# leimao/Voice-Converter-CycleGAN

Measured on NVIDIA H100. Metric: CycleGAN-VC train steps/sec @ batch 256x[24,128] MCEP, higher is better.
Workload: dtype f16f8 (forward / data gradient: fp16 MMA + two e4m3 cross-term MMAs = 2 MMA units per product; weight gradient: fp16 MMA alone, 1 unit; f32 accumulate)

## Files before the change

### voice-converter-cyclegan_b200/csrc/tc_gemm.cu

```cuda
#include "tc_gemm.cuh"
#include "geom.h"
#include "kernels.cuh"
#include "wgmma.cuh"

#include <cuda.h>
#include <stdint.h>
#include <stdio.h>

namespace {

typedef CUresult (*EncodeTiledFn)(CUtensorMap*, CUtensorMapDataType, cuuint32_t, void*, const cuuint64_t*, const cuuint64_t*,
                                  const cuuint32_t*, const cuuint32_t*, CUtensorMapInterleave, CUtensorMapSwizzle,
                                  CUtensorMapL2promotion, CUtensorMapFloatOOBfill);
EncodeTiledFn get_encoder() {
  static EncodeTiledFn fn = nullptr;
  if (!fn) {
    void* p = nullptr; cudaDriverEntryPointQueryResult q;
    if (cudaGetDriverEntryPoint("cuTensorMapEncodeTiled", &p, cudaEnableDefault, &q) == cudaSuccess && q == cudaDriverEntryPointSuccess)
      fn = (EncodeTiledFn)p;
  }
  return fn;
}
bool make_tmap3(CUtensorMap* m, const void* base, uint64_t d0, uint64_t d1, uint64_t d2, uint32_t b1) {
  EncodeTiledFn enc = get_encoder();
  if (!enc) return false;
  cuuint64_t dims[3] = {d0, d1, d2};
  cuuint64_t strides[2] = {d0 * 2, d0 * d1 * 2};
  cuuint32_t box[3] = {64, b1, 1};
  cuuint32_t es[3] = {1, 1, 1};
  return enc(m, CU_TENSOR_MAP_DATA_TYPE_BFLOAT16, 3, const_cast<void*>(base), dims, strides, box, es, CU_TENSOR_MAP_INTERLEAVE_NONE,
             CU_TENSOR_MAP_SWIZZLE_128B, CU_TENSOR_MAP_L2_PROMOTION_L2_256B, CU_TENSOR_MAP_FLOAT_OOB_FILL_NONE) == CUDA_SUCCESS;
}

bool make_tmap3_t(CUtensorMap* m, const void* base, CUtensorMapDataType dt, int esize, uint64_t d0, uint64_t d1, uint64_t d2, uint32_t b0, uint32_t b1) {
  EncodeTiledFn enc = get_encoder();
  if (!enc) return false;
  cuuint64_t dims[3] = {d0, d1, d2};
  cuuint64_t strides[2] = {d0 * (uint64_t)esize, d0 * d1 * (uint64_t)esize};
  cuuint32_t box[3] = {b0, b1, 1};
  cuuint32_t es[3] = {1, 1, 1};
  return enc(m, dt, 3, const_cast<void*>(base), dims, strides, box, es, CU_TENSOR_MAP_INTERLEAVE_NONE,
             b0 * esize == 64 ? CU_TENSOR_MAP_SWIZZLE_64B : CU_TENSOR_MAP_SWIZZLE_128B, CU_TENSOR_MAP_L2_PROMOTION_L2_256B,
             CU_TENSOR_MAP_FLOAT_OOB_FILL_NONE) == CUDA_SUCCESS;
}

__device__ __forceinline__ uint32_t smem_u32(const void* p) { return (uint32_t)__cvta_generic_to_shared(p); }

__device__ __forceinline__ void mbar_init(uint64_t* bar, uint32_t count) {
  asm volatile("mbarrier.init.shared::cta.b64 [%0], %1;" ::"r"(smem_u32(bar)), "r"(count));
}
__device__ __forceinline__ void fence_barrier_init() { asm volatile("fence.mbarrier_init.release.cluster;" ::: "memory"); }
__device__ __forceinline__ void mbar_wait(uint64_t* bar, uint32_t parity) {
  asm volatile(
      "{\n\t"
      ".reg .pred p;\n\t"
      "WAIT_LOOP:\n\t"
      "mbarrier.try_wait.parity.shared::cta.b64 p, [%0], %1;\n\t"
      "@p bra.uni WAIT_DONE;\n\t"
      "bra.uni WAIT_LOOP;\n\t"
      "WAIT_DONE:\n\t"
      "}" ::"r"(smem_u32(bar)), "r"(parity) : "memory");
}
__device__ __forceinline__ void cp_async16(uint32_t dst_smem, const void* src, uint32_t src_bytes) {
  asm volatile("cp.async.cg.shared.global [%0], [%1], 16, %2;" ::"r"(dst_smem), "l"(src), "r"(src_bytes) : "memory");
}
__device__ __forceinline__ void cp_async_arrive_noinc(uint64_t* bar) {
  asm volatile("cp.async.mbarrier.arrive.noinc.shared::cta.b64 [%0];" ::"r"(smem_u32(bar)) : "memory");
}
__device__ __forceinline__ void mbar_expect_tx(uint64_t* bar, uint32_t bytes) {
  asm volatile("mbarrier.arrive.expect_tx.shared::cta.b64 _, [%0], %1;" ::"r"(smem_u32(bar)), "r"(bytes) : "memory");
}
__device__ __forceinline__ void tma_load3(uint32_t dst_smem, const CUtensorMap* map, int c0, int c1, int c2, uint64_t* bar) {
  asm volatile("cp.async.bulk.tensor.3d.shared::cluster.global.tile.mbarrier::complete_tx::bytes [%0], [%1, {%2, %3, %4}], [%5];"
               ::"r"(dst_smem), "l"(map), "r"(c0), "r"(c1), "r"(c2), "r"(smem_u32(bar)) : "memory");
}
__device__ __forceinline__ void tma_prefetch_desc(const CUtensorMap* map) {
  asm volatile("prefetch.tensormap [%0];" ::"l"(map) : "memory");
}
__device__ __forceinline__ void fence_proxy_async() { asm volatile("fence.proxy.async.shared::cta;" ::: "memory"); }
__device__ __forceinline__ uint64_t make_desc(uint32_t smem_addr, uint32_t lbo_bytes, uint32_t sbo_bytes, uint64_t layout = 1) {
  return (uint64_t)((smem_addr >> 4) & 0x3FFF) | ((uint64_t)((lbo_bytes >> 4) & 0x3FFF) << 16) |
         ((uint64_t)((sbo_bytes >> 4) & 0x3FFF) << 32) | (layout << 62);
}
__device__ __forceinline__ uint64_t make_desc64(uint32_t smem_addr) { return make_desc(smem_addr, 16, 512, 2); }
template <int N>
__device__ __forceinline__ void fence_acc(float (&d)[N]) {
#pragma unroll
  for (int i = 0; i < N; ++i) asm volatile("" : "+f"(d[i])::"memory");
}
__device__ __forceinline__ void mbar_arrive(uint64_t* bar) {
  asm volatile("mbarrier.arrive.shared::cta.b64 _, [%0];" ::"r"(smem_u32(bar)) : "memory");
}
__device__ __forceinline__ void consumer_bar() { asm volatile("bar.sync 3, 256;" ::: "memory"); }
__device__ __forceinline__ void st_shared16(uint32_t addr, uint4 v) {
  asm volatile("st.shared.v4.b32 [%0], {%1, %2, %3, %4};" ::"r"(addr), "r"(v.x), "r"(v.y), "r"(v.z), "r"(v.w) : "memory");
}
__device__ __forceinline__ uint4 e4m3x8_to_f16x8(uint2 v) {
  uint32_t w[4];
#pragma unroll
  for (int i = 0; i < 4; ++i) {
    const uint32_t src = (i < 2 ? v.x : v.y) >> (16 * (i & 1));
    const __half2_raw h = __nv_cvt_fp8x2_to_halfraw2((__nv_fp8x2_storage_t)(src & 0xFFFFu), __NV_E4M3);
    w[i] = (uint32_t)h.x | ((uint32_t)h.y << 16);
  }
  return make_uint4(w[0], w[1], w[2], w[3]);
}

struct FastDiv { uint32_t mul, shr, d; };
__host__ inline FastDiv make_fastdiv(uint32_t d) {
  FastDiv f; f.d = d;
  uint32_t l = 0; while ((1ull << l) < d) ++l;
  f.mul = (uint32_t)(((1ull << 32) * ((1ull << l) - d)) / d + 1);
  f.shr = l;
  return f;
}
__device__ __forceinline__ uint32_t fdiv(uint32_t n, const FastDiv& f) { return (uint32_t)(((uint64_t)__umulhi(n, f.mul) + n) >> f.shr); }

__device__ __forceinline__ uint32_t sw128(int r, int c) { return (uint32_t)((r >> 3) * 1024 + (r & 7) * 128 + ((c ^ (r & 7)) << 4)); }

struct TcNTParams {
  GatherGeom g;
  const __nv_bfloat16 *a_hi, *a_lo; int a_ld; int C;
  const __nv_bfloat16 *b_hi, *b_lo; int Nw;
  int N;
  int n_tiles;
  int debug;
  float* dst; int d_ld; const float* bias; int accumulate;
  int perm; int Cc;
  int R;
  const float *gamma_a, *beta_a, *gamma_g, *beta_g;
  float* stats;
  const float* resid;
  float* y; __nv_bfloat16 *y_hi, *y_lo;
  int C_out;
  const float* bp; int bp_ld;
  __nv_bfloat16 *dp_hi, *dp_lo; int dp_ld;
  float *dbeta_a, *dgamma_a, *dbeta_g, *dgamma_g;
  CUtensorMap tm_b_hi, tm_b_lo;
  const uint8_t *a8_hi, *a8_lo;
  CUtensorMap tm_b8_hi, tm_b8_lo;
  uint8_t* y8;
  PackGeom pk;
  FastDiv div_bw, div_w;
};

struct RowPos { int b, y, x; };
__device__ __forceinline__ RowPos nt_row(const TcNTParams& p, long long m) {
  RowPos r;
  r.y = (int)fdiv((uint32_t)m, p.div_bw);
  const uint32_t rem = (uint32_t)m - (uint32_t)r.y * p.div_bw.d;
  r.b = (int)fdiv(rem, p.div_w);
  r.x = (int)(rem - (uint32_t)r.b * p.div_w.d);
  return r;
}
__device__ __forceinline__ uint32_t nt_tile_taps(const TcNTParams& p, long long m0, long long M) {
  const long long m1 = m0 + 127 < M ? m0 + 127 : M - 1;
  return gather_tap_mask(p.g, nt_row(p, m0).y, nt_row(p, m1).y);
}

struct TcTNParams {
  GatherGeom g;
  const __nv_bfloat16 *x_hi, *x_lo; int x_ld; int C;
  const __nv_bfloat16 *g_hi, *g_lo; int g_ld; int N;
  float* dw_a; float* dw_g; int n_split;
  int ksplit;
  FastDiv div_hw, div_w;
  CUtensorMap tm_g_hi, tm_g_lo;
  const uint8_t *x8_hi, *x8_lo;
  const uint8_t *g8_hi, *g8_lo;
  int w16;
  int fold_n;
  float* part; long long part_k, numel_a;
};

__device__ __forceinline__ float* tn_dst(float* base, int slab, int C, int c, int ncols, int col, int fold_n) {
  if (fold_n) { const int t = col / fold_n; return base + ((long long)t * C + c) * fold_n + (col - t * fold_n); }
  return base + ((long long)slab * C + c) * ncols + col;
}

constexpr int kProducerThreads = 128;


template <int BN, int NPL>
struct NTCfg {
  static constexpr int A_PLANE = 128 * 128;
  static constexpr int B_PLANE = BN * 128;
  static constexpr int PLANES = NPL == 2 ? 2 : 1;
  static constexpr int STAGE = PLANES * (A_PLANE + B_PLANE);
  static constexpr int STAGES = (192 * 1024) / STAGE;
  static constexpr int SMEM = STAGES * STAGE + 1024;
  static_assert(STAGES * STAGE >= 128 * BN * 4, "the finished fp32 tile is staged over the pipeline stages");
};

template <int BN>
__device__ __forceinline__ int acc_off(int r, int n) { return r * BN + (n & ~31) + ((((n >> 2) & 7) ^ (r & 7)) << 2) + (n & 3); }
template <int BN>
__device__ __forceinline__ void acc_ld32(const float* acc, int r, int col, uint32_t (&v)[32]) {
#pragma unroll
  for (int c = 0; c < 8; ++c) {
    const float4 x = *reinterpret_cast<const float4*>(acc + r * BN + col + ((c ^ (r & 7)) << 2));
    v[4 * c] = __float_as_uint(x.x); v[4 * c + 1] = __float_as_uint(x.y); v[4 * c + 2] = __float_as_uint(x.z); v[4 * c + 3] = __float_as_uint(x.w);
  }
}

__device__ __forceinline__ float warp_colsum32(float (&t)[32], int lane) {
#pragma unroll
  for (int o = 16, n = 32; o >= 1; o >>= 1, n >>= 1) {
    const bool up = (lane & o) != 0;
#pragma unroll
    for (int i = 0; i < n / 2; ++i) {
      float send = up ? t[i] : t[i + n / 2];
      float keep = up ? t[i + n / 2] : t[i];
      t[i] = keep + __shfl_xor_sync(0xffffffffu, send, o);
    }
  }
  return t[0];
}
__device__ __forceinline__ void epi_bar(int id) { asm volatile("bar.sync %0, 128;" ::"r"(id) : "memory"); }

__device__ __forceinline__ float sample_sum(float v, float (*xch)[32], int q, int lane, int spw, int barid) {
  if (spw == 1) return v;
  epi_bar(barid);
  xch[q][lane] = v;
  epi_bar(barid);
  const int q0 = (q / spw) * spw;
  float r = 0.f;
  for (int w = 0; w < spw; ++w) r += xch[q0 + w][lane];
  return r;
}
__device__ __forceinline__ void bc4(const float* p, float (&v)[4]) { const float4 x = *reinterpret_cast<const float4*>(p); v[0] = x.x; v[1] = x.y; v[2] = x.z; v[3] = x.w; }
__device__ __forceinline__ float fast_sigmoid(float x) { return __fdividef(1.f, 1.f + __expf(-x)); }
__device__ __forceinline__ void chunk_norm_coeffs(const float (&v)[32], const float* __restrict__ gamma, const float* __restrict__ beta,
                                                  int ch, int R, float (*xch)[32], float* bc, int q, int lane, int spw, int barid, float& mean, float& rstd) {
  float t[32];
#pragma unroll
  for (int k = 0; k < 32; ++k) t[k] = v[k];
  float s = warp_colsum32(t, lane);
  s = sample_sum(s, xch, q, lane, spw, barid);
  mean = s / (float)R;
  __syncwarp();
  bc[lane] = mean;
  __syncwarp();
#pragma unroll
  for (int k = 0; k < 32; k += 4) {
    float4 m4 = *reinterpret_cast<const float4*>(bc + k);
    float d0 = v[k] - m4.x, d1 = v[k + 1] - m4.y, d2 = v[k + 2] - m4.z, d3 = v[k + 3] - m4.w;
    t[k] = d0 * d0; t[k + 1] = d1 * d1; t[k + 2] = d2 * d2; t[k + 3] = d3 * d3;
  }
  float ss = warp_colsum32(t, lane);
  ss = sample_sum(ss, xch, q, lane, spw, barid);
  rstd = 1.f / sqrtf(ss / (float)R + 1e-6f);
  const float sc = rstd * gamma[ch + lane];
  const float of = beta[ch + lane] - mean * sc;
  __syncwarp();
  bc[lane] = sc; bc[32 + lane] = of;
  __syncwarp();
}

__device__ __forceinline__ void pair_norm_coeffs(const float (&v0)[32], const float (&v1)[32], const float* __restrict__ gamma, const float* __restrict__ beta,
                                                 int ch, int R, float (*xch)[32], float* bc, int q, int lane, int spw, int barid, float& mean, float& rstd) {
  float t[32];
#pragma unroll
  for (int k = 0; k < 32; ++k) t[k] = v0[k] + v1[k];
  float s = warp_colsum32(t, lane);
  s = sample_sum(s, xch, q, lane, spw, barid);
  const float inv = 1.f / (float)(2 * R);
  mean = s * inv;
  __syncwarp();
  bc[lane] = mean;
  __syncwarp();
#pragma unroll
  for (int k = 0; k < 32; k += 4) {
    float4 m4 = *reinterpret_cast<const float4*>(bc + k);
    const float m[4] = {m4.x, m4.y, m4.z, m4.w};
#pragma unroll
    for (int j = 0; j < 4; ++j) { const float d0 = v0[k + j] - m[j], d1 = v1[k + j] - m[j]; t[k + j] = fmaf(d0, d0, d1 * d1); }
  }
  float ss = warp_colsum32(t, lane);
  ss = sample_sum(ss, xch, q, lane, spw, barid);
  rstd = 1.f / sqrtf(ss * inv + 1e-6f);
  const float sc = rstd * gamma[ch + lane];
  const float of = beta[ch + lane] - mean * sc;
  __syncwarp();
  bc[lane] = sc; bc[32 + lane] = of;
  __syncwarp();
}

__device__ __forceinline__ uint32_t hp_off(int r, int c) { return (uint32_t)(r * 16 + ((c ^ ((r >> 1) & 3)) << 2)); }
template <class F>
__device__ __forceinline__ void rows_out(float* stg, const float (&o)[32], int lane, F f) {
  const int hc = lane & 3, hr = lane >> 2;
#pragma unroll
  for (int h = 0; h < 2; ++h) {
    __syncwarp();
#pragma unroll
    for (int c = 0; c < 4; ++c)
      *reinterpret_cast<float4*>(stg + hp_off(lane, c)) = make_float4(o[16 * h + 4 * c], o[16 * h + 4 * c + 1], o[16 * h + 4 * c + 2], o[16 * h + 4 * c + 3]);
    __syncwarp();
#pragma unroll
    for (int i = 0; i < 4; ++i) {
      const int rr = hr + 8 * i;
      f(rr, 16 * h + 4 * hc, *reinterpret_cast<const float4*>(stg + hp_off(rr, hc)));
    }
  }
}
__device__ __forceinline__ void rows_in(float* stg, float (&v)[32], int lane, const float4 (&pre)[8]) {
  const int hc = lane & 3, hr = lane >> 2;
#pragma unroll
  for (int h = 0; h < 2; ++h) {
    __syncwarp();
#pragma unroll
    for (int i = 0; i < 4; ++i) *reinterpret_cast<float4*>(stg + hp_off(hr + 8 * i, hc)) = pre[4 * h + i];
    __syncwarp();
#pragma unroll
    for (int c = 0; c < 4; ++c) {
      const float4 x = *reinterpret_cast<const float4*>(stg + hp_off(lane, c));
      v[16 * h + 4 * c] = x.x; v[16 * h + 4 * c + 1] = x.y; v[16 * h + 4 * c + 2] = x.z; v[16 * h + 4 * c + 3] = x.w;
    }
// ... 454 lines not shown
  const bool n_fast = g.Hy > 1;

  if (threadIdx.x == 0) {
    for (int s = 0; s < S; ++s) { mbar_init(&full_bar[s], kProducerThreads + 1); mbar_init(&empty_bar[s], 8); }
    mbar_init(&acc_free_bar, 8);
    fence_barrier_init();
    tma_prefetch_desc(&p.tm_b_hi);
    if (NPL == 2) tma_prefetch_desc(&p.tm_b_lo);
    if (NPL == 3) { tma_prefetch_desc(&p.tm_b8_hi); tma_prefetch_desc(&p.tm_b8_lo); }
  }
  __syncthreads();

  if (warp < 4) {
    const int t = threadIdx.x;
    const int chunk = t & 7, rsub = t >> 3;
    int stage = 0; uint32_t phase = 0;
    int it = 0;
    for (int tile = blockIdx.x; tile < num_tiles; tile += gridDim.x, ++it) {
      const long long m0 = (long long)(n_fast ? tile / n_tiles : tile % m_tiles) * 128;
      const int n0 = (n_fast ? tile % n_tiles : tile / m_tiles) * BN;
      if (EPI != 0 && it > 0) mbar_wait(&acc_free_bar, (uint32_t)(it - 1) & 1u);
      const uint32_t taps = nt_tile_taps(p, m0, M);
      int rb[8], ry[8], rx[8];
#pragma unroll
      for (int i = 0; i < 8; ++i) {
        long long m = m0 + rsub + 16 * i;
        if (m < M) {
          if constexpr (PK) {
            const int dout = p.pk.div * g.sx;
            const int u = pack_find(p.pk.off, p.pk.n, m * dout);
            const long long o0 = __ldg(p.pk.off + u), o1 = __ldg(p.pk.off + u + 1);
            rb[i] = (int)(o0 / p.pk.div); ry[i] = (int)((o1 - o0) / p.pk.div); rx[i] = (int)(m - o0 / dout) * g.sx;
          } else {
            const RowPos o = nt_row(p, m);
            rb[i] = o.b; ry[i] = o.y * g.sy; rx[i] = o.x * g.sx;
          }
        } else { rb[i] = -1; ry[i] = 0; rx[i] = 0; }
      }
      for (int pass = 0; pass < (NPL == 3 ? 2 : 1); ++pass)
      for (int tap = 0; tap < g.ntaps; ++tap) {
        if (!((taps >> tap) & 1u)) continue;
        long long aoff[8];
#pragma unroll
        for (int i = 0; i < 8; ++i) {
          const int cofs = NPL == 3 && pass == 0 ? (chunk & 3) * 16 : chunk * 8;
          if constexpr (PK) {
            const int xx = rx[i] + g.ox[tap];
            aoff[i] = rb[i] >= 0 && xx >= 0 && xx < ry[i] ? (long long)(rb[i] + xx) * p.a_ld + cofs : -1;
          } else {
            int yy = ry[i] + g.oy[tap], xx = rx[i] + g.ox[tap];
            bool ok = rb[i] >= 0 && yy >= 0 && yy < g.Hs && xx >= 0 && xx < g.Ws;
            aoff[i] = ok ? ((long long)(rb[i] * g.Hs + yy) * g.Ws + xx) * p.a_ld + cofs : -1;
          }
        }
        for (int cc = 0; cc < cchunks; ++cc) {
          const int c0 = cc << 6;
          mbar_wait(&empty_bar[stage], phase ^ 1);
          const uint32_t sA = smem_base + stage * Cfg::STAGE;
          const uint32_t sB = sA + Cfg::PLANES * Cfg::A_PLANE;
          if (t == 0) {
            mbar_expect_tx(&full_bar[stage], Cfg::PLANES * Cfg::B_PLANE);
            if (NPL == 3) {
              if (pass == 0) {
                tma_load3(sB, &p.tm_b8_hi, c0, n0, g.widx[tap], &full_bar[stage]);
                tma_load3(sB + Cfg::B_PLANE / 2, &p.tm_b8_lo, c0, n0, g.widx[tap], &full_bar[stage]);
              } else {
                tma_load3(sB, &p.tm_b_hi, c0, n0, g.widx[tap], &full_bar[stage]);
              }
            } else {
              tma_load3(sB, &p.tm_b_hi, c0, n0, g.widx[tap], &full_bar[stage]);
              if (NPL == 2) tma_load3(sB + Cfg::B_PLANE, &p.tm_b_lo, c0, n0, g.widx[tap], &full_bar[stage]);
            }
          }
          if (!(p.debug & 4)) {
#pragma unroll
            for (int i = 0; i < 8; ++i) {
              const int r = rsub + 16 * i;
              const uint32_t so = sw128(r, chunk);
              const bool ok = aoff[i] >= 0;
              const long long off = ok ? aoff[i] + c0 : 0;
              if (NPL == 3) {
                if (pass == 0)
                  cp_async16(sA + so, (chunk < 4 ? p.a8_hi : p.a8_lo) + off, ok ? 16u : 0u);
                else
                  cp_async16(sA + so, p.a_hi + off, ok ? 16u : 0u);
              } else {
                cp_async16(sA + so, p.a_hi + off, ok ? 16u : 0u);
                if (NPL == 2) cp_async16(sA + Cfg::A_PLANE + so, p.a_lo + off, ok ? 16u : 0u);
              }
            }
          }
          cp_async_arrive_noinc(&full_bar[stage]);
          if (++stage == S) { stage = 0; phase ^= 1; }
        }
      }
    }
  } else {
    const int cw = warp - 4;
    const int wg = cw >> 2;
    const int tw = threadIdx.x - 128 * (wg + 1);
    float* acc_s = reinterpret_cast<float*>(smem_raw + (smem_base - smem_u32(smem_raw)));
    int stage = 0; uint32_t phase = 0;
    for (int tile = blockIdx.x; tile < num_tiles; tile += gridDim.x) {
      const long long m0 = (long long)(n_fast ? tile / n_tiles : tile % m_tiles) * 128;
      const int n0 = (n_fast ? tile % n_tiles : tile / m_tiles) * BN;
      float d[BN / 2];
#pragma unroll
      for (int i = 0; i < BN / 2; ++i) d[i] = 0.f;
      int prev = -1;
      const int kb_pass = __popc(nt_tile_taps(p, m0, M)) * cchunks;
      if constexpr (NPL == 3) {
        consume_stages<BN, MMA_E4M3_CROSS, 0, Cfg>(d, kb_pass, stage, phase, prev, full_bar, empty_bar, smem_base, wg, lane);
        rescale_acc(d, 1.f / (float)(1 << CGVC_Q_ACC_SHIFT));
        consume_stages<BN, MMA_F16, 0, Cfg>(d, kb_pass, stage, phase, prev, full_bar, empty_bar, smem_base, wg, lane);
      } else {
        consume_stages<BN, NPL == 2 ? MMA_BF16X3 : MMA_BF16, 0, Cfg>(d, kb_pass, stage, phase, prev, full_bar, empty_bar, smem_base, wg, lane);
      }
      wgmma_wait<0>();
      fence_acc(d);
      if (prev >= 0 && lane == 0) mbar_arrive(&empty_bar[prev]);
      const int r0 = wg * 64 + (tw >> 5) * 16 + ((tw & 31) >> 2), c0 = 2 * (tw & 3);
      if constexpr (EPI == 0) {
        if (!(p.debug & 3)) nt_store_fragments<BN>(p, d, M, m0, n0, r0, c0);
      } else {
        consumer_bar();
        if (!(p.debug & 2)) {
#pragma unroll
          for (int j = 0; j < BN / 8; ++j) {
            *reinterpret_cast<float2*>(acc_s + acc_off<BN>(r0, 8 * j + c0)) = make_float2(d[4 * j], d[4 * j + 1]);
            *reinterpret_cast<float2*>(acc_s + acc_off<BN>(r0 + 8, 8 * j + c0)) = make_float2(d[4 * j + 2], d[4 * j + 3]);
          }
        }
        consumer_bar();
        nt_tile_epilogue<BN, NPL, EPI>(p, M, m0, n0, cw & 3, lane, epi_stage[cw], epi_rowp[cw], epi_bc[cw], epi_xch[wg], acc_s, wg, 2);
        fence_proxy_async();
        __syncwarp();
        if (lane == 0) mbar_arrive(&acc_free_bar);
      }
    }
  }
}

#define CGVC_Q_WGRAD_SHIFT 12
template <int NPL, int W16>
struct TNCfg {
  static constexpr int A_PLANE = 64 * 256;
  static constexpr int B_PLANE = 64 * 512;
  static constexpr int PLANES = (NPL == 1 || W16) ? 1 : 2;
  static constexpr int STAGE = PLANES * (A_PLANE + B_PLANE);
  static constexpr int STAGES = (192 * 1024) / STAGE;
  static constexpr int SMEM = STAGES * STAGE + 1024;
};

template <int NPL, int W16, int DET>
__global__ void __launch_bounds__(kNTThreads, 1)
tc_gg_tn_kernel(const __grid_constant__ TcTNParams p) {
  static_assert(W16 == 0 || NPL == 3, "the fp16-only weight gradient is a form of CGVC_PREC_F16F8");
  using Cfg = TNCfg<NPL, W16>;
  constexpr int S = Cfg::STAGES;
  constexpr int BN = 256;
  extern __shared__ uint8_t smem_raw[];
  __shared__ __align__(8) uint64_t full_bar[S], empty_bar[S];

  const uint32_t smem_base = (smem_u32(smem_raw) + 1023u) & ~1023u;
  const int warp = threadIdx.x >> 5, lane = threadIdx.x & 31;
  const GatherGeom& g = p.g;
  const long long M = (long long)g.B * g.Hy * g.Wx;
  const int HW = g.Hy * g.Wx;
  const int n_tiles = (p.g_ld + BN - 1) / BN, c_tiles = (p.x_ld + 127) / 128;
  const int num_items = n_tiles * c_tiles * g.ntaps * p.ksplit;
  constexpr int pass0 = (NPL == 3 && !W16) ? 0 : 1;
  long long chunk_rows = (M + p.ksplit - 1) / p.ksplit;
  chunk_rows = (chunk_rows + 63) / 64 * 64;

  struct Item { int n0, c0, tap, ks; long long mbeg, mend; int num_kb; };
  auto decode = [&](int item) -> Item {
    Item w;
    int n_t = item % n_tiles; int t1 = item / n_tiles;
    int c_t = t1 % c_tiles; int t2 = t1 / c_tiles;
    w.tap = t2 % g.ntaps; const int ks = t2 / g.ntaps; w.ks = ks;
    w.n0 = n_t * BN; w.c0 = c_t * 128;
    w.mbeg = (long long)ks * chunk_rows;
    w.mend = (w.mbeg + chunk_rows < M) ? w.mbeg + chunk_rows : M;
    w.num_kb = w.mend > w.mbeg ? (int)((w.mend - w.mbeg + 63) / 64) : 0;
    return w;
  };

  if (threadIdx.x == 0) {
    for (int s = 0; s < S; ++s) { mbar_init(&full_bar[s], kProducerThreads + 1); mbar_init(&empty_bar[s], 8); }
    fence_barrier_init();
    tma_prefetch_desc(&p.tm_g_hi);
    if (NPL == 2) tma_prefetch_desc(&p.tm_g_lo);
  }
  __syncthreads();

  if (warp < 4) {
    const int t = threadIdx.x;
    const int chunk = t & 7, rsub = t >> 3;
    int stage = 0; uint32_t phase = 0;
    for (int item = blockIdx.x; item < num_items; item += gridDim.x) {
      const Item w = decode(item);
      for (int pass = pass0; pass < 2; ++pass)
      for (int kb = 0; kb < w.num_kb; ++kb) {
        mbar_wait(&empty_bar[stage], phase ^ 1);
        const uint32_t sA = smem_base + stage * Cfg::STAGE;
        const uint32_t sB = sA + Cfg::PLANES * Cfg::A_PLANE;
        long long xoff[4];
#pragma unroll
        for (int i = 0; i < 4; ++i) {
          const long long m = w.mbeg + (long long)kb * 64 + rsub + 16 * i;
          xoff[i] = -1;
          if (m < w.mend) {
            const uint32_t mu = (uint32_t)m;
            int b = (int)fdiv(mu, p.div_hw); int rem = (int)(mu - (uint32_t)b * (uint32_t)HW);
            int y = (int)fdiv((uint32_t)rem, p.div_w); int x = rem - y * g.Wx;
            int yy = y * g.sy + g.oy[w.tap], xx = x * g.sx + g.ox[w.tap];
            if (yy >= 0 && yy < g.Hs && xx >= 0 && xx < g.Ws)
              xoff[i] = ((long long)(b * g.Hs + yy) * g.Ws + xx) * p.x_ld + w.c0 + chunk * 8;
          }
        }
        if (NPL == 3 && pass == 0) {
#pragma unroll
          for (int i = 0; i < 4; ++i) {
            const int kr = rsub + 16 * i;
            const uint32_t so = sw128(kr, chunk);
#pragma unroll
            for (int a = 0; a < 2; ++a) {
              const bool ok = xoff[i] >= 0 && (w.c0 + a * 64) < p.x_ld;
              uint2 vh = make_uint2(0u, 0u), vl = make_uint2(0u, 0u);
              if (ok) { vh = __ldg(reinterpret_cast<const uint2*>(p.x8_hi + xoff[i] + a * 64)); vl = __ldg(reinterpret_cast<const uint2*>(p.x8_lo + xoff[i] + a * 64)); }
              st_shared16(sA + a * 8192 + so, e4m3x8_to_f16x8(vh));
              st_shared16(sA + Cfg::A_PLANE + a * 8192 + so, e4m3x8_to_f16x8(vl));
            }
            const long long m = w.mbeg + (long long)kb * 64 + kr;
#pragma unroll
            for (int a = 0; a < 4; ++a) {
              const int col = w.n0 + a * 64 + chunk * 8;
              const bool ok = m < w.mend && col < p.g_ld;
              uint2 vh = make_uint2(0u, 0u), vl = make_uint2(0u, 0u);
              if (ok) { vh = __ldg(reinterpret_cast<const uint2*>(p.g8_hi + m * p.g_ld + col)); vl = __ldg(reinterpret_cast<const uint2*>(p.g8_lo + m * p.g_ld + col)); }
              st_shared16(sB + a * 8192 + so, e4m3x8_to_f16x8(vh));
              st_shared16(sB + Cfg::B_PLANE + a * 8192 + so, e4m3x8_to_f16x8(vl));
            }
          }
          fence_proxy_async();
          if (t == 0) mbar_expect_tx(&full_bar[stage], 0);
          mbar_arrive(&full_bar[stage]);
        } else {
          if (t == 0) {
            const int row0 = (int)(w.mbeg + (long long)kb * 64);
            int natoms = 0;
#pragma unroll
            for (int a = 0; a < 4; ++a) natoms += (w.n0 + a * 64) < p.g_ld ? 1 : 0;
            mbar_expect_tx(&full_bar[stage], (NPL == 2 ? 2 : 1) * natoms * 8192);
#pragma unroll
            for (int a = 0; a < 4; ++a) {
              if ((w.n0 + a * 64) < p.g_ld) {
                tma_load3(sB + a * 8192, &p.tm_g_hi, w.n0 + a * 64, row0, 0, &full_bar[stage]);
                if (NPL == 2) tma_load3(sB + Cfg::B_PLANE + a * 8192, &p.tm_g_lo, w.n0 + a * 64, row0, 0, &full_bar[stage]);
              }
            }
          }
#pragma unroll
          for (int i = 0; i < 4; ++i) {
            const uint32_t so = sw128(rsub + 16 * i, chunk);
#pragma unroll
            for (int a = 0; a < 2; ++a) {
              const bool ok = xoff[i] >= 0 && (w.c0 + a * 64) < p.x_ld;
              const long long off = ok ? xoff[i] + a * 64 : 0;
              cp_async16(sA + a * 8192 + so, p.x_hi + off, ok ? 16u : 0u);
              if (NPL == 2) cp_async16(sA + Cfg::A_PLANE + a * 8192 + so, p.x_lo + off, ok ? 16u : 0u);
            }
          }
          cp_async_arrive_noinc(&full_bar[stage]);
        }
        if (++stage == S) { stage = 0; phase ^= 1; }
      }
    }
  } else {
    const int cw = warp - 4;
    const int wg = cw >> 2;
    const int tw = threadIdx.x - 128 * (wg + 1);
    int stage = 0; uint32_t phase = 0;
    for (int item = blockIdx.x; item < num_items; item += gridDim.x) {
      const Item w = decode(item);
      if (w.num_kb == 0) continue;
      float d[BN / 2];
#pragma unroll
      for (int i = 0; i < BN / 2; ++i) d[i] = 0.f;
      int prev = -1;
      if constexpr (NPL == 3 && !W16) {
        consume_stages<BN, MMA_F16_CROSS, 1, Cfg>(d, w.num_kb, stage, phase, prev, full_bar, empty_bar, smem_base, wg, lane);
        rescale_acc(d, 1.f / (float)(1 << CGVC_Q_WGRAD_SHIFT));
        consume_stages<BN, MMA_F16, 1, Cfg>(d, w.num_kb, stage, phase, prev, full_bar, empty_bar, smem_base, wg, lane);
      } else if constexpr (NPL == 3) {
        consume_stages<BN, MMA_F16, 1, Cfg>(d, w.num_kb, stage, phase, prev, full_bar, empty_bar, smem_base, wg, lane);
      } else {
        consume_stages<BN, NPL == 2 ? MMA_BF16X3 : MMA_BF16, 1, Cfg>(d, w.num_kb, stage, phase, prev, full_bar, empty_bar, smem_base, wg, lane);
      }
      wgmma_wait<0>();
      fence_acc(d);
      if (lane == 0) mbar_arrive(&empty_bar[prev]);
      const int c = w.c0 + wg * 64 + (tw >> 5) * 16 + ((tw & 31) >> 2);
#pragma unroll
      for (int j = 0; j < BN / 8; ++j) {
        const int n = w.n0 + 8 * j + 2 * (tw & 3);
        if (n >= p.N) continue;
        float* base; int nn; int ncols;
        if (n < p.n_split) { base = DET ? p.part + w.ks * p.part_k : p.dw_a; nn = n; ncols = p.n_split; }
        else { base = DET ? p.part + w.ks * p.part_k + p.numel_a : p.dw_g; nn = n - p.n_split; ncols = p.N - p.n_split; }
#pragma unroll
        for (int h = 0; h < 2; ++h) {
          if (c + 8 * h >= p.C) continue;
          float* dst = tn_dst(base, g.widx[w.tap], p.C, c + 8 * h, ncols, nn, p.fold_n);
          if constexpr (DET) asm volatile("st.global.v2.f32 [%0], {%1, %2};" ::"l"(dst), "f"(d[4 * j + 2 * h]), "f"(d[4 * j + 2 * h + 1]) : "memory");
          else asm volatile("red.global.add.v2.f32 [%0], {%1, %2};" ::"l"(dst), "f"(d[4 * j + 2 * h]), "f"(d[4 * j + 2 * h + 1]) : "memory");
        }
      }
    }
  }
}

__host__ __device__ __forceinline__ int perm_row(int perm, int co, int cout, int noff) {
  if (perm == 1) return (co >> 7) * 256 + (noff ? 128 : 0) + (co & 127);
  if (perm == 2) { const int Ch = cout >> 1; const int s = co >= Ch ? 1 : 0; const int c = co - s * Ch; return (c >> 6) * 256 + (noff ? 128 : 0) + s * 64 + (c & 63); }
  return noff + co;
}
__host__ __device__ __forceinline__ long long w_src(int tap, int ci, int co, int cin, int cout, int fold_n) {
  if (fold_n) { const int t = co / fold_n; return ((long long)t * cin + ci) * fold_n + (co - t * fold_n); }
  return ((long long)tap * cin + ci) * cout + co;
}
__global__ void __launch_bounds__(256)
prep_weights_kernel(const float* __restrict__ w, int taps, int cin, int cout, int nt_n, int cin_k, int cin_n, int nt_k, int noff, int perm, int fold_n,
                    __nv_bfloat16* __restrict__ wf_hi, __nv_bfloat16* __restrict__ wf_lo,
                    __nv_bfloat16* __restrict__ wd_hi, __nv_bfloat16* __restrict__ wd_lo) {
  __shared__ float tile[32][33];
  const int tap = blockIdx.z;
  const int ci0 = blockIdx.y * 32, co0 = blockIdx.x * 32;
  const int tx = threadIdx.x & 31, ty = threadIdx.x >> 5;
  for (int r = ty; r < 32; r += 8) {
    int ci = ci0 + r, co = co0 + tx;
    float v = 0.f;
    if (ci < cin && co < cout) {
      v = w[w_src(tap, ci, co, cin, cout, fold_n)];
      __nv_bfloat16 h = __float2bfloat16_rn(v);
      __nv_bfloat16 l = __float2bfloat16_rn(v - __bfloat162float(h));
      long long o = ((long long)tap * cin_n + ci) * nt_k + noff + co;
      wd_hi[o] = h; wd_lo[o] = l;
    }
    tile[r][tx] = v;
  }
  __syncthreads();
  for (int r = ty; r < 32; r += 8) {
    int co = co0 + r, ci = ci0 + tx;
    if (ci < cin && co < cout) {
      float v = tile[tx][r];
      __nv_bfloat16 h = __float2bfloat16_rn(v);
      __nv_bfloat16 l = __float2bfloat16_rn(v - __bfloat162float(h));
      const int nrow = perm_row(perm, co, cout, noff);
      long long o = ((long long)tap * nt_n + nrow) * cin_k + ci;
      wf_hi[o] = h; wf_lo[o] = l;
    }
  }
}

__global__ void copy_bias_kernel(const float* __restrict__ b, float* __restrict__ dst, int n, int noff, int perm) {
  int i = blockIdx.x * 256 + threadIdx.x;
  if (i < n) dst[perm_row(perm, i, n, noff)] = b[i];
}

__global__ void __launch_bounds__(256)
prep_weights_q_kernel(const float* __restrict__ w, int taps, int cin, int cout, int nt_n, int cin_q, int noff, int perm, int fold_n,
                      __half* __restrict__ q16, uint8_t* __restrict__ q8hi, uint8_t* __restrict__ q8lo) {
  const int cq = cin / 4;
  const long long total = (long long)taps * cout * cq;
  for (long long i = (long long)blockIdx.x * 256 + threadIdx.x; i < total; i += (long long)gridDim.x * 256) {
    const int c4 = (int)(i % cq); long long r = i / cq;
    const int co = (int)(r % cout); const int tap = (int)(r / cout);
    const int ci = c4 * 4;
    float v[4];
#pragma unroll
    for (int k = 0; k < 4; ++k) v[k] = w[w_src(tap, ci + k, co, cin, cout, fold_n)];
    const int nrow = perm_row(perm, co, cout, noff);
    const long long o = ((long long)tap * nt_n + nrow) * cin_q + ci;
    uint2 hh; uint32_t b_hi, b_lo;
    cgvc_quant4(v, CGVC_Q_W_SHI, CGVC_Q_W_SLO, hh, b_hi, b_lo);
    *reinterpret_cast<uint2*>(q16 + o) = hh;
    *reinterpret_cast<uint32_t*>(q8hi + o) = b_hi;
    *reinterpret_cast<uint32_t*>(q8lo + o) = b_lo;
  }
}

__global__ void __launch_bounds__(256)
prep_weights_qd_kernel(const float* __restrict__ w, int taps, int cin, int cout, int cin_n, int nt_q, int noff, int fold_n,
                       __half* __restrict__ q16, uint8_t* __restrict__ q8hi, uint8_t* __restrict__ q8lo) {
  const int cq = cout / 4;
  const long long total = (long long)taps * cin * cq;
  for (long long i = (long long)blockIdx.x * 256 + threadIdx.x; i < total; i += (long long)gridDim.x * 256) {
    const int c4 = (int)(i % cq); long long r = i / cq;
    const int ci = (int)(r % cin); const int tap = (int)(r / cin);
    const float4 v4 = *reinterpret_cast<const float4*>(w + w_src(tap, ci, c4 * 4, cin, cout, fold_n));
    const float v[4] = {v4.x, v4.y, v4.z, v4.w};
    const long long o = ((long long)tap * cin_n + ci) * nt_q + noff + c4 * 4;
    uint2 hh; uint32_t b_hi, b_lo;
    cgvc_quant4(v, CGVC_Q_W_SHI, CGVC_Q_W_SLO, hh, b_hi, b_lo);
    *reinterpret_cast<uint2*>(q16 + o) = hh;
    *reinterpret_cast<uint32_t*>(q8hi + o) = b_hi;
    *reinterpret_cast<uint32_t*>(q8lo + o) = b_lo;
  }
}

struct PrepJob {
  long long w_off, b_off;
  int taps, cin, cout, nt_n, cin_q, cin_n, nt_q, noff, perm, fold_n;
  __half* q16; uint8_t *q8hi, *q8lo;
  __half* dq16; uint8_t *dq8hi, *dq8lo;
  float* bias;
  int tiles_ci, tiles_co;
  int first_block;
};

__global__ void __launch_bounds__(256)
prep_weights_q_all_kernel(const float* __restrict__ params, const PrepJob* __restrict__ jobs, int j0, int j1, int block0) {
  __shared__ float tile[32][65];
  const int blk = (int)blockIdx.x + block0;
  int lo = j0, hi = j1 - 1;
  while (lo < hi) { const int mid = (lo + hi + 1) >> 1; if (jobs[mid].first_block <= blk) lo = mid; else hi = mid - 1; }
  const PrepJob& J = jobs[lo];
  int r = blk - J.first_block;
  const int tco = r % J.tiles_co; r /= J.tiles_co;
  const int tci = r % J.tiles_ci; const int tap = r / J.tiles_ci;
  const int ci0 = tci * 32, co0 = tco * 64;
  const float* __restrict__ w = params + J.w_off;
  const int t = threadIdx.x;
  {
    const int c4 = (t & 15) * 4;
    for (int rr = t >> 4; rr < 32; rr += 16) {
      const int ci = ci0 + rr, co = co0 + c4;
      float v[4] = {0.f, 0.f, 0.f, 0.f};
      if (ci < J.cin && co < J.cout) {
        const float4 q = *reinterpret_cast<const float4*>(w + w_src(tap, ci, co, J.cin, J.cout, J.fold_n));
        v[0] = q.x; v[1] = q.y; v[2] = q.z; v[3] = q.w;
        if (J.dq16) {
          const long long o = ((long long)tap * J.cin_n + ci) * J.nt_q + J.noff + co;
          uint2 hh; uint32_t b_hi, b_lo;
          cgvc_quant4(v, CGVC_Q_W_SHI, CGVC_Q_W_SLO, hh, b_hi, b_lo);
          *reinterpret_cast<uint2*>(J.dq16 + o) = hh;
          *reinterpret_cast<uint32_t*>(J.dq8hi + o) = b_hi;
          *reinterpret_cast<uint32_t*>(J.dq8lo + o) = b_lo;
        }
      }
      tile[rr][c4] = v[0]; tile[rr][c4 + 1] = v[1]; tile[rr][c4 + 2] = v[2]; tile[rr][c4 + 3] = v[3];
    }
  }
  __syncthreads();
  {
    const int lane = t & 31, warp = t >> 5;
    const int cig = (lane & 3) * 8;
    const int col = warp * 8 + (lane >> 2);
    const int co = co0 + col;
    if (co < J.cout && ci0 + cig < J.cin_q) {
      float va[4], vb[4];
#pragma unroll
      for (int k = 0; k < 4; ++k) { va[k] = tile[cig + k][col]; vb[k] = tile[cig + 4 + k][col]; }
      const int nrow = perm_row(J.perm, co, J.cout, J.noff);
      const long long o = ((long long)tap * J.nt_n + nrow) * J.cin_q + ci0 + cig;
      uint2 ha, hb; uint32_t a_hi, a_lo, b_hi, b_lo;
      cgvc_quant4(va, CGVC_Q_W_SHI, CGVC_Q_W_SLO, ha, a_hi, a_lo);
      cgvc_quant4(vb, CGVC_Q_W_SHI, CGVC_Q_W_SLO, hb, b_hi, b_lo);
      *reinterpret_cast<uint4*>(J.q16 + o) = make_uint4(ha.x, ha.y, hb.x, hb.y);
      *reinterpret_cast<uint2*>(J.q8hi + o) = make_uint2(a_hi, b_hi);
      *reinterpret_cast<uint2*>(J.q8lo + o) = make_uint2(a_lo, b_lo);
    }
  }
  if (tap == 0 && tci == 0 && tco == 0 && J.b_off >= 0)
    for (int i = t; i < J.cout; i += 256) J.bias[perm_row(J.perm, i, J.cout, J.noff)] = params[J.b_off + i];
}

template <class K>
cudaError_t set_smem(K kernel, int bytes) {
  static std::vector<const void*> done;
  const void* key = (const void*)kernel;
  for (const void* d : done) if (d == key) return cudaSuccess;
  cudaError_t e = cudaFuncSetAttribute(kernel, cudaFuncAttributeMaxDynamicSharedMemorySize, bytes);
  if (e == cudaSuccess) done.push_back(key);
  return e;
}

struct ProfRec { cudaEvent_t a, b; double flops; int cls; long long M; int N, K; };
int g_tc_debug = 0;
int g_tc_prep_batched = 1;
bool g_prof_on = false;
std::vector<ProfRec> g_prof;
void prof_begin(cudaStream_t st, double flops, int cls, long long M = 0, int N = 0, int K = 0) {
  if (!g_prof_on) return;
  ProfRec r; r.flops = flops; r.cls = cls; r.M = M; r.N = N; r.K = K;
  cudaEventCreate(&r.a); cudaEventCreate(&r.b);
  cudaEventRecord(r.a, st);
  g_prof.push_back(r);
}
void prof_end(cudaStream_t st) { if (g_prof_on && !g_prof.empty()) cudaEventRecord(g_prof.back().b, st); }

inline int tile_rows(int n_real, int n_padded) { return (n_padded % 256 == 0) ? 256 : (n_real <= 32 ? 32 : 128); }

int num_sms() {
  static int n = 0;
  if (!n) { int dev = 0; cudaGetDevice(&dev); cudaDeviceGetAttribute(&n, cudaDevAttrMultiProcessorCount, dev); }
  return n;
}

cudaError_t launch_nt(TcNTParams p, int precision, cudaStream_t st, int epi) {
  const long long M = (long long)p.g.B * p.g.Hy * p.g.Wx;
  if (M == 0) return cudaSuccess;
  if (M >= (1ll << 31)) return cudaErrorInvalidValue;
  const bool x3 = precision == 1;
  if (p.g.ntaps == 0) return cudaErrorInvalidValue;
  p.div_bw = make_fastdiv((uint32_t)(p.g.B * p.g.Wx)); p.div_w = make_fastdiv((uint32_t)p.g.Wx);
  const int bn = tile_rows(p.N, p.Nw);
  p.n_tiles = bn == 32 ? 1 : p.Nw / bn;
  const long long tiles = ((M + 127) / 128) * p.n_tiles;
  dim3 grid((unsigned)(tiles < num_sms() ? tiles : num_sms()));
  cudaError_t e;
  ++g_cgvc_launches;
  p.debug = g_tc_debug;
  prof_begin(st, 2.0 * (double)M * p.N * p.g.ntaps * p.C, (epi == 1 || epi == 2 || epi == 5) ? 2 : 0, M, p.N, p.g.ntaps * p.C);
#define LAUNCH_NT(BN_, NPL_, EPI_, ...)                                                                        \
  do {                                                                                                         \
    e = set_smem(tc_gg_nt_kernel<BN_, NPL_, EPI_, ##__VA_ARGS__>, NTCfg<BN_, NPL_>::SMEM);                     \
    if (e != cudaSuccess) return e;                                                                            \
    tc_gg_nt_kernel<BN_, NPL_, EPI_, ##__VA_ARGS__><<<grid, kNTThreads, NTCfg<BN_, NPL_>::SMEM, st>>>(p);      \
  } while (0)
  if (epi != 0 && bn != 256) return cudaErrorInvalidValue;
  if (p.pk.off) {
    if (epi != 0 || p.g.B != 1 || p.g.Hy != 1) return cudaErrorInvalidValue;
    const int npl = precision == 3 ? 3 : x3 ? 2 : 1;
    if (bn == 256)      { if (npl == 3) LAUNCH_NT(256, 3, 0, true); else if (npl == 2) LAUNCH_NT(256, 2, 0, true); else LAUNCH_NT(256, 1, 0, true); }
    else if (bn == 128) { if (npl == 3) LAUNCH_NT(128, 3, 0, true); else if (npl == 2) LAUNCH_NT(128, 2, 0, true); else LAUNCH_NT(128, 1, 0, true); }
    else                { if (npl == 3) LAUNCH_NT(32, 3, 0, true);  else if (npl == 2) LAUNCH_NT(32, 2, 0, true);  else LAUNCH_NT(32, 1, 0, true); }
  }
  else if (precision == 3) {
    if (epi == 1)       LAUNCH_NT(256, 3, 1);
    else if (epi == 2)  LAUNCH_NT(256, 3, 2);
    else if (epi == 5)  LAUNCH_NT(256, 3, 5);
    else if (epi != 0)  return cudaErrorInvalidValue;
    else if (bn == 256) LAUNCH_NT(256, 3, 0);
    else if (bn == 128) LAUNCH_NT(128, 3, 0);
    else                LAUNCH_NT(32, 3, 0);
  }
  else if (epi == 1)  { if (x3) LAUNCH_NT(256, 2, 1); else LAUNCH_NT(256, 1, 1); }
  else if (epi == 2)  { if (x3) LAUNCH_NT(256, 2, 2); else LAUNCH_NT(256, 1, 2); }
  else if (epi == 3)  { if (x3) LAUNCH_NT(256, 2, 3); else LAUNCH_NT(256, 1, 3); }
  else if (epi == 4)  { if (x3) LAUNCH_NT(256, 2, 4); else LAUNCH_NT(256, 1, 4); }
  else if (epi == 5)  { if (x3) LAUNCH_NT(256, 2, 5); else LAUNCH_NT(256, 1, 5); }
  else if (bn == 256) { if (x3) LAUNCH_NT(256, 2, 0); else LAUNCH_NT(256, 1, 0); }
  else if (bn == 128) { if (x3) LAUNCH_NT(128, 2, 0); else LAUNCH_NT(128, 1, 0); }
  else                { if (x3) LAUNCH_NT(32, 2, 0);  else LAUNCH_NT(32, 1, 0); }
#undef LAUNCH_NT
  prof_end(st);
  return cudaGetLastError();
}

cudaError_t launch_tn(TcTNParams p, int precision, cudaStream_t st, const DetSlab* det) {
  const long long M = (long long)p.g.B * p.g.Hy * p.g.Wx;
  if (M == 0) return cudaSuccess;
  if (M >= (1ll << 31)) return cudaErrorInvalidValue;
  const int tiles = ((p.g_ld + 255) / 256) * ((p.x_ld + 127) / 128) * p.g.ntaps;
  const int nsm = num_sms();
  long long maxsplit = M / 1024; if (maxsplit < 1) maxsplit = 1; if (maxsplit > 32) maxsplit = 32;
  int ksplit = 1; double best = 0.0;
  for (int ks = 1; ks <= (int)maxsplit; ++ks) {
    long long items = (long long)tiles * ks;
    double eff = (double)items / (double)(((items + nsm - 1) / nsm) * nsm);
    if (items < nsm) eff *= 0.5;
    if (eff > best + 0.02) { best = eff; ksplit = ks; }
  }
  const long long numel = (long long)p.g.ntaps * p.C * p.N;
  auto chunk_of = [&](int ks) { return ((M + ks - 1) / ks + 63) / 64 * 64; };
  if (det && det->p)
    while (ksplit > 1 && ((long long)ksplit * numel > det->cap || (long long)(ksplit - 1) * chunk_of(ksplit) >= M)) --ksplit;
  const bool det_split = det && det->p && ksplit > 1;
  if (det_split) { p.part = det->p; p.part_k = numel; p.numel_a = (long long)p.g.ntaps * p.C * p.n_split; }
  p.ksplit = ksplit;
  p.div_hw = make_fastdiv((uint32_t)(p.g.Hy * p.g.Wx)); p.div_w = make_fastdiv((uint32_t)p.g.Wx);
  const long long items = (long long)tiles * ksplit;
  dim3 grid((unsigned)(items < nsm ? items : nsm));
  cudaError_t e;
  ++g_cgvc_launches;
  prof_begin(st, 2.0 * (double)M * p.N * p.g.ntaps * p.C, 1, M, p.N, p.g.ntaps * p.C);
#define LAUNCH_TN(NPL_, W16_, DET_)                                                               \
  do {                                                                                            \
    e = set_smem(tc_gg_tn_kernel<NPL_, W16_, DET_>, TNCfg<NPL_, W16_>::SMEM);                     \
    if (e != cudaSuccess) return e;                                                               \
    tc_gg_tn_kernel<NPL_, W16_, DET_><<<grid, kNTThreads, TNCfg<NPL_, W16_>::SMEM, st>>>(p);      \
  } while (0)
  if (det_split) {
    if (precision == 3) { if (p.w16) LAUNCH_TN(3, 1, 1); else LAUNCH_TN(3, 0, 1); }
    else if (precision == 1) LAUNCH_TN(2, 0, 1);
    else                     LAUNCH_TN(1, 0, 1);
  } else {
    if (precision == 3) { if (p.w16) LAUNCH_TN(3, 1, 0); else LAUNCH_TN(3, 0, 0); }
    else if (precision == 1) LAUNCH_TN(2, 0, 0);
    else                     LAUNCH_TN(1, 0, 0);
  }
#undef LAUNCH_TN
  prof_end(st);
  if (!det_split) return cudaGetLastError();
  e = cudaGetLastError();
  if (e != cudaSuccess) return e;
  return launch_reduce_parts(p.part, ksplit, numel, DetSegs{{p.dw_a, p.dw_g}, {0, p.numel_a}, {p.numel_a, p.dw_g ? numel - p.numel_a : 0}}, st);
}

inline int ru(int v, int m) { return (v + m - 1) / m * m; }
inline int Ntot(const TcLayer& L) { return L.cout * (L.gated ? 2 : 1); }
inline int cin_k(const TcLayer& L) { return ru(L.cin, 64); }
inline int cin_n(const TcLayer& L) { return ru(L.cin, 128); }
inline int nt_k(const TcLayer& L) { return ru(Ntot(L), 64); }
inline int nt_n(const TcLayer& L) { return ru(Ntot(L), 128); }
inline int cin_q(const TcLayer& L) { return ru(L.cin, 128); }
inline int nt_q(const TcLayer& L) { return ru(Ntot(L), 128); }
inline size_t wq_elems(const TcLayer& L) { return (size_t)L.kh * L.kw * nt_n(L) * cin_q(L); }
inline size_t wdq_elems(const TcLayer& L) { return (size_t)L.kh * L.kw * cin_n(L) * nt_q(L); }
inline size_t wf_elems(const TcLayer& L) { return (size_t)L.kh * L.kw * nt_n(L) * cin_k(L); }
inline size_t wd_elems(const TcLayer& L) { return (size_t)L.kh * L.kw * cin_n(L) * nt_k(L); }
inline int layer_perm(const TcLayer& L) {
  if (L.gated && L.shuffle == 2 && L.cout % 128 == 0) return 2;
  return (L.gated && L.cout % 128 == 0) ? 1 : 0;
}
inline bool layer_ok(const TcLayer& L) {
  if (L.fold && (L.gated || L.kh * L.kw != 1 || L.cout % L.fold || (L.cout / L.fold) % 4)) return false;
  return L.kh * L.kw <= CGVC_MAX_TAPS && Ntot(L) % 4 == 0;
}
inline bool layer_ok_q(const TcLayer& L) { return layer_ok(L) && L.cin % 4 == 0; }


bool make_layer_maps(TcLayer& L) {
  const int taps = L.kh * L.kw;
  const int bf = tile_rows(Ntot(L), nt_n(L)), bd = tile_rows(L.cin, cin_n(L));
  return make_tmap3(&L.tm_f_hi, L.wf_hi, cin_k(L), nt_n(L), taps, bf) &&
         make_tmap3(&L.tm_f_lo, L.wf_lo, cin_k(L), nt_n(L), taps, bf) &&
         make_tmap3(&L.tm_d_hi, L.wd_hi, nt_k(L), cin_n(L), taps, bd) &&
         make_tmap3(&L.tm_d_lo, L.wd_lo, nt_k(L), cin_n(L), taps, bd);
}

bool make_layer_maps_q(TcLayer& L) {
  const int taps = L.kh * L.kw;
  const int bf = tile_rows(Ntot(L), nt_n(L)), bd = tile_rows(L.cin, cin_n(L));
  const CUtensorMapDataType F16 = CU_TENSOR_MAP_DATA_TYPE_FLOAT16, U8 = CU_TENSOR_MAP_DATA_TYPE_UINT8;
  bool ok = make_tmap3_t(&L.tm_q16, L.wq16, F16, 2, cin_q(L), nt_n(L), taps, 64, bf) &&
            make_tmap3_t(&L.tm_q8hi, L.wq8hi, U8, 1, cin_q(L), nt_n(L), taps, 64, bf) &&
            make_tmap3_t(&L.tm_q8lo, L.wq8lo, U8, 1, cin_q(L), nt_n(L), taps, 64, bf);
  if (ok && L.wdq16)
    ok = make_tmap3_t(&L.tm_dq16, L.wdq16, F16, 2, nt_q(L), cin_n(L), taps, 64, bd) &&
         make_tmap3_t(&L.tm_dq8hi, L.wdq8hi, U8, 1, nt_q(L), cin_n(L), taps, 64, bd) &&
         make_tmap3_t(&L.tm_dq8lo, L.wdq8lo, U8, 1, nt_q(L), cin_n(L), taps, 64, bd);
  return ok;
}


int refresh_layer(TcLayer& L, const float* ka, const float* kg, const float* ba, const float* bg, cudaStream_t st) {
  const int taps = L.kh * L.kw;
  dim3 grid((L.cout + 31) / 32, (L.cin + 31) / 32, taps);
  g_cgvc_launches += L.gated ? 4 : 2;
  const int perm = layer_perm(L);
  const int fn = L.fold ? L.cout / L.fold : 0;
  if (!L.wq16) prep_weights_kernel<<<grid, 256, 0, st>>>(ka, taps, L.cin, L.cout, nt_n(L), cin_k(L), cin_n(L), nt_k(L), 0, perm, fn, L.wf_hi, L.wf_lo, L.wd_hi, L.wd_lo);
  if (!L.fold) copy_bias_kernel<<<(L.cout + 255) / 256, 256, 0, st>>>(ba, L.bias, L.cout, 0, perm);
  if (L.gated) {
    if (!L.wq16) prep_weights_kernel<<<grid, 256, 0, st>>>(kg, taps, L.cin, L.cout, nt_n(L), cin_k(L), cin_n(L), nt_k(L), L.cout, perm, fn, L.wf_hi, L.wf_lo, L.wd_hi, L.wd_lo);
    copy_bias_kernel<<<(L.cout + 255) / 256, 256, 0, st>>>(bg, L.bias, L.cout, L.cout, perm);
  }
  if (L.wq16) {
    long long tot = (long long)taps * L.cout * (L.cin / 4); long long nb = (tot + 255) / 256; if (nb > num_sms() * 32) nb = num_sms() * 32;
    g_cgvc_launches += L.gated ? 2 : 1;
    prep_weights_q_kernel<<<(unsigned)nb, 256, 0, st>>>(ka, taps, L.cin, L.cout, nt_n(L), cin_q(L), 0, perm, fn, (__half*)L.wq16, L.wq8hi, L.wq8lo);
    if (L.gated) prep_weights_q_kernel<<<(unsigned)nb, 256, 0, st>>>(kg, taps, L.cin, L.cout, nt_n(L), cin_q(L), L.cout, perm, fn, (__half*)L.wq16, L.wq8hi, L.wq8lo);
    if (L.wdq16) {
      g_cgvc_launches += L.gated ? 2 : 1;
      prep_weights_qd_kernel<<<(unsigned)nb, 256, 0, st>>>(ka, taps, L.cin, L.cout, cin_n(L), nt_q(L), 0, fn, (__half*)L.wdq16, L.wdq8hi, L.wdq8lo);
      if (L.gated) prep_weights_qd_kernel<<<(unsigned)nb, 256, 0, st>>>(kg, taps, L.cin, L.cout, cin_n(L), nt_q(L), L.cout, fn, (__half*)L.wdq16, L.wdq8hi, L.wdq8lo);
    }
  }
  return (int)cudaGetLastError();
}

int layer_fwd(const TcLayer& L, int precision, const __nv_bfloat16* xhi, const __nv_bfloat16* xlo, int n, int H, int W, int sh, int sw,
              float* P, cudaStream_t st, const TcFuse* fuse = nullptr, bool* fused_out = nullptr, const PackGeom* pk = nullptr) {
  if (!layer_ok(L) || (precision == 3 && !layer_ok_q(L))) return TC_UNSUPPORTED;
  if (pk && (n != 1 || H != 1 || L.kh != 1 || fuse)) return (int)cudaErrorInvalidValue;
  TcNTParams p; memset(&p, 0, sizeof p);
  p.g = fwd_geom(n, H, W, L.kh, L.kw, sh, sw);
  if (pk) p.pk = *pk;
  p.a_hi = xhi; p.a_lo = xlo; p.a_ld = cin_k(L); p.C = cin_k(L);
  p.b_hi = L.wf_hi; p.b_lo = L.wf_lo; p.Nw = nt_n(L); p.N = Ntot(L);
  p.dst = P; p.d_ld = Ntot(L); p.bias = L.bias; p.accumulate = 0;
  p.perm = layer_perm(L); p.Cc = L.cout;
  p.tm_b_hi = L.tm_f_hi; p.tm_b_lo = L.tm_f_lo;
  if (precision == 3) {
    if (!L.wq16) return TC_UNSUPPORTED;
    p.a_ld = cin_q(L); p.C = cin_q(L); p.a_lo = nullptr;
    p.a8_hi = reinterpret_cast<const uint8_t*>(xlo); p.a8_lo = p.a8_hi + (size_t)n * H * W * cin_q(L);
    p.tm_b_hi = L.tm_q16; p.tm_b8_hi = L.tm_q8hi; p.tm_b8_lo = L.tm_q8lo;
  }
  int epi = 0;
  if (fuse && fuse->R > 0) {
    const bool shape_ok = H == 1 && (fuse->R == 32 || fuse->R == 64 || fuse->R == 128) && p.g.Wx == fuse->R && nt_n(L) % 256 == 0 && Ntot(L) == nt_n(L);
    if (shape_ok && L.gated && p.perm == 1) epi = 1; else if (shape_ok && L.gated && p.perm == 2) epi = 5; else if (shape_ok && !L.gated) epi = 2;
    if (epi) {
      p.R = fuse->R; p.gamma_a = fuse->gamma_a; p.beta_a = fuse->beta_a; p.gamma_g = fuse->gamma_g; p.beta_g = fuse->beta_g;
      p.stats = fuse->stats; p.resid = fuse->resid; p.y = fuse->y; p.y_hi = fuse->y_hi; p.y_lo = fuse->y_lo;
      p.y8 = reinterpret_cast<uint8_t*>(fuse->y_lo);
      p.C_out = epi == 5 ? L.cout / 2 : (L.gated ? L.cout : Ntot(L));
      if (!p.y_hi || (epi == 2 && !p.resid)) epi = 0;
    }
  }
  if (fused_out) *fused_out = epi != 0;
  if (!epi && !P) return (int)cudaErrorInvalidValue;
  return (int)launch_nt(p, precision, st, epi);
}

int layer_dgrad(const TcLayer& L, int precision, const __nv_bfloat16* dPhi, const __nv_bfloat16* dPlo, int n, int H, int W, int sh, int sw,
                float* dx, int accumulate, cudaStream_t st, const TcBwdFuse* fuse = nullptr, bool* fused_out = nullptr) {
  if (fused_out) *fused_out = false;
  if (!layer_ok(L) || (precision == 3 && (!layer_ok_q(L) || !L.wdq16))) return TC_UNSUPPORTED;
  std::vector<GatherGeom> gs = dgrad_geoms(n, H, W, L.kh, L.kw, sh, sw);
  for (const GatherGeom& g : gs) if (g.ntaps == 0) return TC_UNSUPPORTED;
  int epi = 0;
  if (fuse && fuse->R > 0 && gs.size() == 1 && H == 1 && sh == 1 && sw == 1 && (fuse->R == 32 || fuse->R == 64 || fuse->R == 128) &&
      gs[0].Wx == fuse->R && cin_n(L) % 256 == 0 && L.cin == cin_n(L) && fuse->bp && fuse->stats && fuse->dp_hi && fuse->dp_lo && fuse->gamma_a &&
      (fuse->gated ? (fuse->gamma_g && fuse->beta_a && fuse->beta_g) : (dx != nullptr)) && precision != 3)
    epi = fuse->gated ? 3 : 4;
  for (const GatherGeom& g : gs) {
    TcNTParams p; memset(&p, 0, sizeof p);
    p.g = g;
    p.a_hi = dPhi; p.a_lo = dPlo; p.a_ld = nt_k(L); p.C = nt_k(L);
    p.b_hi = L.wd_hi; p.b_lo = L.wd_lo; p.Nw = cin_n(L); p.N = L.cin;
// ... 409 lines not shown
```

Baseline: 10.02.

## Schedule weight-gradient GEMM work as whole tiles plus split-K tail

In the non-deterministic weight-gradient kernel, each CTA now handles whole output tiles over the full reduction range for as many rounds as evenly fill the grid. Only the leftover tiles are split along K, in contiguous k-chunk ranges spread across CTAs. The goal is fewer atomic reductions into the fp32 gradient buffers and fewer accumulator drains, while keeping load balance in the tail. It also adds a debug flag that can skip the epilogue stores, and the deterministic split path keeps the old round-robin order.

```diff
diff --git a/voice-converter-cyclegan_b200/csrc/tc_gemm.cu b/voice-converter-cyclegan_b200/csrc/tc_gemm.cu
--- a/voice-converter-cyclegan_b200/csrc/tc_gemm.cu
+++ b/voice-converter-cyclegan_b200/csrc/tc_gemm.cu
@@ -164,6 +164,7 @@
   const __nv_bfloat16 *g_hi, *g_lo; int g_ld; int N;
   float* dw_a; float* dw_g; int n_split;
   int ksplit;
+  int debug;
   FastDiv div_hw, div_w;
   CUtensorMap tm_g_hi, tm_g_lo;
   const uint8_t *x8_hi, *x8_lo;
@@ -924,6 +925,39 @@
   static constexpr int SMEM = STAGES * STAGE + 1024;
 };
 
+template <int DET>
+struct TNWalk {
+  int tiles, ksplit, whole, rem, q, i, pos, end;
+  __device__ TNWalk(int tiles_, int ksplit_) : tiles(tiles_), ksplit(ksplit_), whole(0), rem(0), q(1), i(0) {
+    const int b = blockIdx.x, G = gridDim.x;
+    if (DET) { pos = b; end = tiles * ksplit; return; }
+    whole = tiles / G;
+    rem = tiles - whole * G;
+    const int n = rem * ksplit, base = n / G, extra = n - base * G;
+    q = min(ksplit, base + (extra ? 1 : 0));
+    pos = b * base + min(b, extra);
+    end = pos + base + (b < extra ? 1 : 0);
+  }
+  __device__ bool next(int& tile, int& k0, int& k1) {
+    if (DET) {
+      if (pos >= end) return false;
+      tile = pos % tiles; k0 = pos / tiles; k1 = k0 + 1;
+      pos += gridDim.x;
+      return true;
+    }
+    if (i < whole) { tile = i * gridDim.x + blockIdx.x; k0 = 0; k1 = ksplit; ++i; return true; }
+    if (pos >= end) return false;
+    const int blk = pos / (rem * q), off = pos - blk * rem * q;
+    const int len = min(q, ksplit - blk * q);
+    const int r = off / len, c = off - r * len;
+    tile = whole * gridDim.x + r;
+    k0 = blk * q + c;
+    k1 = k0 + min(len - c, end - pos);
+    pos += k1 - k0;
+    return true;
+  }
+};
+
 template <int NPL, int W16, int DET>
 __global__ void __launch_bounds__(kNTThreads, 1)
 tc_gg_tn_kernel(const __grid_constant__ TcTNParams p) {
@@ -940,20 +974,20 @@
   const long long M = (long long)g.B * g.Hy * g.Wx;
   const int HW = g.Hy * g.Wx;
   const int n_tiles = (p.g_ld + BN - 1) / BN, c_tiles = (p.x_ld + 127) / 128;
-  const int num_items = n_tiles * c_tiles * g.ntaps * p.ksplit;
+  const int num_tiles = n_tiles * c_tiles * g.ntaps;
   constexpr int pass0 = (NPL == 3 && !W16) ? 0 : 1;
   long long chunk_rows = (M + p.ksplit - 1) / p.ksplit;
   chunk_rows = (chunk_rows + 63) / 64 * 64;
 
   struct Item { int n0, c0, tap, ks; long long mbeg, mend; int num_kb; };
-  auto decode = [&](int item) -> Item {
+  auto decode = [&](int tile, int k0, int k1) -> Item {
     Item w;
-    int n_t = item % n_tiles; int t1 = item / n_tiles;
-    int c_t = t1 % c_tiles; int t2 = t1 / c_tiles;
-    w.tap = t2 % g.ntaps; const int ks = t2 / g.ntaps; w.ks = ks;
+    int n_t = tile % n_tiles; int t1 = tile / n_tiles;
+    int c_t = t1 % c_tiles;
+    w.tap = t1 / c_tiles; w.ks = k0;
     w.n0 = n_t * BN; w.c0 = c_t * 128;
-    w.mbeg = (long long)ks * chunk_rows;
-    w.mend = (w.mbeg + chunk_rows < M) ? w.mbeg + chunk_rows : M;
+    w.mbeg = (long long)k0 * chunk_rows;
+    w.mend = ((long long)k1 * chunk_rows < M) ? (long long)k1 * chunk_rows : M;
     w.num_kb = w.mend > w.mbeg ? (int)((w.mend - w.mbeg + 63) / 64) : 0;
     return w;
   };
@@ -970,8 +1004,9 @@
     const int t = threadIdx.x;
     const int chunk = t & 7, rsub = t >> 3;
     int stage = 0; uint32_t phase = 0;
-    for (int item = blockIdx.x; item < num_items; item += gridDim.x) {
-      const Item w = decode(item);
+    TNWalk<DET> walk(num_tiles, p.ksplit);
+    for (int tile, k0, k1; walk.next(tile, k0, k1);) {
+      const Item w = decode(tile, k0, k1);
       for (int pass = pass0; pass < 2; ++pass)
       for (int kb = 0; kb < w.num_kb; ++kb) {
         mbar_wait(&empty_bar[stage], phase ^ 1);
@@ -1054,8 +1089,9 @@
     const int wg = cw >> 2;
     const int tw = threadIdx.x - 128 * (wg + 1);
     int stage = 0; uint32_t phase = 0;
-    for (int item = blockIdx.x; item < num_items; item += gridDim.x) {
-      const Item w = decode(item);
+    TNWalk<DET> walk(num_tiles, p.ksplit);
+    for (int tile, k0, k1; walk.next(tile, k0, k1);) {
+      const Item w = decode(tile, k0, k1);
       if (w.num_kb == 0) continue;
       float d[BN / 2];
 #pragma unroll
@@ -1073,6 +1109,7 @@
       wgmma_wait<0>();
       fence_acc(d);
       if (lane == 0) mbar_arrive(&empty_bar[prev]);
+      if (p.debug & 8) continue;
       const int c = w.c0 + wg * 64 + (tw >> 5) * 16 + ((tw & 31) >> 2);
 #pragma unroll
       for (int j = 0; j < BN / 8; ++j) {
@@ -1353,6 +1390,7 @@
   const bool det_split = det && det->p && ksplit > 1;
   if (det_split) { p.part = det->p; p.part_k = numel; p.numel_a = (long long)p.g.ntaps * p.C * p.n_split; }
   p.ksplit = ksplit;
+  p.debug = g_tc_debug;
   p.div_hw = make_fastdiv((uint32_t)(p.g.Hy * p.g.Wx)); p.div_w = make_fastdiv((uint32_t)p.g.Wx);
   const long long items = (long long)tiles * ksplit;
   dim3 grid((unsigned)(items < nsm ? items : nsm));
```

After: 10.15 (median of 6 runs). 1.01x the previous value.
